# bluenote-1577/skani

Hardware: AMD Instinct MI355X
Metric: genome-pairs/sec (triangle, ~5 Mbp genomes) (higher is better)
Workload: dtype u64

## Files before the change

skani_amd/csrc/chain.hip:

```cpp
#include <algorithm>
#include <cmath>

#include "internal.h"

namespace skh {

#include "chain_types.h"
#include "chain_join.h"
#include "chain_chunk.h"
#include "chain_dp.h"
#include "chain_select.h"
#include "chain_stats.h"
#include "chain_estimate.h"

namespace {

static void genome_halves(const skh_sketch_set* S) {
    std::lock_guard<std::mutex> lk(S->cache_mu);
    if (S->halves.size() == S->n_genomes && S->n_genomes) return;
    S->halves.resize(S->n_genomes);
    for (uint32_t g = 0; g < S->n_genomes; g++) {
        skh_sketch_set::GenomeHalf& h = S->halves[g];
        h.n_pos = (uint32_t)(S->pos_off[g + 1] - S->pos_off[g]); h.pos0 = (uint32_t)S->pos_off[g];
        h.seed = S->p_seed.p + S->pos_off[g]; h.g = S->p_g.p + S->pos_off[g]; h.rep = S->p_rep.p; h.salt = S->salt[g];
// ... 230 lines not shown
            check_launch("join_fill");
        }
        std::vector<uint32_t> pa0(np + 1, 0), pc0(np + 1, 0), pi0(np + 1, 0), ps0(np + 1, 0);
        for (uint32_t i = 0; i < np; i++) {
            const uint32_t an = pair_anch[p0 + i];
            pa0[i + 1] = pa0[i] + an;
            pc0[i + 1] = pc0[i] + (an ? std::min(job.chunk_bound[p0 + i], an) : 0);
            const uint32_t icap = an / MIN_ANCHORS;
            pi0[i + 1] = pi0[i] + icap; ps0[i + 1] = ps0[i] + (icap >= big_min ? icap : 0);
            if (ps0[i + 1] < ps0[i]) throw Error("too many candidate intervals in one chain batch");
        }
        const uint32_t NC = pc0[np], NI = pi0[np], NS = ps0[np];
        std::vector<uint32_t> pfx(4 * ((size_t)np + 1));
        memcpy(pfx.data(), pa0.data(), ((size_t)np + 1) * 4); memcpy(pfx.data() + (np + 1), pc0.data(), ((size_t)np + 1) * 4);
        memcpy(pfx.data() + 2 * ((size_t)np + 1), pi0.data(), ((size_t)np + 1) * 4); memcpy(pfx.data() + 3 * ((size_t)np + 1), ps0.data(), ((size_t)np + 1) * 4);
        uint32_t* d_pa0 = upload(ctx, pfx); uint32_t* d_pc0 = d_pa0 + (np + 1); uint32_t* d_pi0 = d_pc0 + (np + 1); uint32_t* d_ps0 = d_pi0 + (np + 1);
        tr.mark("join_fill (+slots)");
        Co *anc_q, *anc_r;
        if constexpr (W::wide) {
            anc_q = ctx->arena.get<uint64_t>((size_t)NA + 16); anc_r = ctx->arena.get<uint64_t>((size_t)NA + 16);
            if (NA) {
                SKH_LAUNCH(widen_anchors_kernel, (NA + 255) / 256, 256, 0, ctx->stream, NA, np, (const uint32_t*)d_pa0, d_wide, (const uint32_t*)anc_q32, (const uint32_t*)anc_r32, anc_q, anc_r);
                check_launch("widen_anchors");
            }
        } else { anc_q = anc_q32; anc_r = anc_r32; }
        Chunk* chunks = ctx->arena.get<Chunk>(NC + 1); uint32_t* chunk_pair = ctx->arena.get<uint32_t>(NC + 1);
        uint32_t* n_chunks = ctx->arena.get<uint32_t>(np);
        SKH_LAUNCH(chunk_kernel<W>, (np + 3) / 4, 256, 0, ctx->stream, np, d_pairs, d_wide, (const uint32_t*)d_pa0, (const uint32_t*)(d_pair_anch + p0),
                   (const uint32_t*)d_pc0, (const Co*)anc_q, chunks, chunk_pair, n_chunks, d_err);
        check_launch("chunk");
        tr.mark("chunk");
        Interval* ivls = ctx->arena.get<Interval>(NI + 1); uint32_t* ivl_cnt = ctx->arena.get<uint32_t>(np);
        uint32_t* ivl_next = ctx->arena.get<uint32_t>(NI + 1); uint32_t* greedy_scratch = ctx->arena.get<uint32_t>((size_t)NS * GREEDY_BIG_WORDS + 1);
        uint32_t* chunk_head = ctx->arena.get<uint32_t>(NC + 1); uint32_t* n_acc = ctx->arena.get<uint32_t>(np);
        FillRegions stage_fills; stage_fills.add(ivl_cnt, np, 0u); stage_fills.add(chunk_head, (uint64_t)NC + 1, 0xFFFFFFFFu);
        bool stage_filled = false;
        const EmitCtxT<W> ec{anc_q, anc_r, d_pairs, d_wide, d_pc0, d_pi0, ivl_cnt, ivls, d_err};
        if (NC) {
            bool chained = false;
            if (band <= (W::wide ? 40u : 84u) && !(W::wide && ctx->tune.wide_sweep_dp)) {
                chained = true;
                constexpr int T = 64;
                const unsigned gt = (NC + T - 1) / T;
                const uint32_t ls = ctx->tune.chain_dp_lds_slots <= 1 ? 1u : 8u;
                const size_t n_spill = band + 1 > ls ? (size_t)(band + 1 - ls) * gt * T : 1;
                unsigned long long* spill_best = ctx->arena.get<unsigned long long>(n_spill); uint32_t* spill_rr = ctx->arena.get<uint32_t>(n_spill);
                uint4* emit_q = ctx->arena.get<uint4>((size_t)DP_EMIT_Q * gt * T);
                const unsigned ob = (NC + DP_ORDER_BLOCK - 1) / DP_ORDER_BLOCK;
                uint32_t* order = ctx->arena.get<uint32_t>(NC); uint32_t* ohist = ctx->arena.get<uint32_t>(2 * DP_ORDER_KEYS);
                stage_fills.add(ohist, 2 * DP_ORDER_KEYS, 0u); fill_regions(ctx, stage_fills); stage_filled = true;
                SKH_LAUNCH(dp_order_hist_kernel, ob, 256, 0, ctx->stream, NC, (const Chunk*)chunks, ohist);
                SKH_LAUNCH(dp_order_scatter_kernel, ob, 256, 0, ctx->stream, NC, (const Chunk*)chunks, (const uint32_t*)ohist, ohist + DP_ORDER_KEYS, order);
                check_launch("dp_order");
#define SKH_DPT2(NB, LS, EX) SKH_LAUNCH((chain_dp_thread_kernel<NB, T, LS, EX, W>), gt, T, 0, ctx->stream, NC, (const Chunk*)chunks, (const uint32_t*)chunk_pair, (const uint32_t*)order, band, ec, spill_best, spill_rr, emit_q, ls == 1 ? 1u : (uint32_t)DP_EMIT_Q)
#define SKH_DPT(NB, EX) do { if (ls == 1) SKH_DPT2(NB, 1, EX); else SKH_DPT2(NB, 8, EX); } while (0)
                if (band == 12) SKH_DPT(12, true); else if (band == 20) SKH_DPT(20, true); else if (band == 35) SKH_DPT(35, true);
                else if (band <= 12) SKH_DPT(12, false); else if (band <= 20) SKH_DPT(20, false); else if (band <= 28) SKH_DPT(28, false); else if (band <= 40) SKH_DPT(40, false);
                else if constexpr (!W::wide) { if (band == 83) SKH_DPT(83, true); else SKH_DPT(84, false); }
#undef SKH_DPT
#undef SKH_DPT2
                check_launch("chain_dp_thread");
            }
            if (!chained) {
                fill_regions(ctx, stage_fills); stage_filled = true;
                unsigned long long* best = ctx->arena.get<unsigned long long>((size_t)NA + 64);
                dzero(best, ((uint64_t)NA + 64) * 8, ctx->stream);
                const unsigned gb = (NC + 3) / 4;
                uint32_t* dp_state = band > 256 ? ctx->arena.get<uint32_t>(3 * (size_t)NA + 4) : nullptr;
#define SKH_DP(PB) SKH_LAUNCH((chain_dp_kernel<PB, W>), gb, 256, 0, ctx->stream, NC, (const Chunk*)chunks, band, (const Co*)anc_q, (const Co*)anc_r, best, dp_state)
                if (band <= 64) SKH_DP(1); else if (band <= 128) SKH_DP(2); else if (band <= 192) SKH_DP(3); else if (band <= 256) SKH_DP(4); else SKH_DP(0);
#undef SKH_DP
                check_launch("chain_dp");
                SKH_LAUNCH(interval_emit_kernel<W>, (NC + 3) / 4, 256, 0, ctx->stream, NC, (const Chunk*)chunks, (const unsigned long long*)best,
                           (const uint32_t*)chunk_pair, ec);
                check_launch("interval_emit");
            }
        }
        if (!stage_filled) fill_regions(ctx, stage_fills);
#define SKH_GREEDY(CAP) SKH_LAUNCH(greedy_fast_kernel<CAP>, np, 64, 0, ctx->stream, np, (const uint32_t*)g_order, (const uint32_t*)d_pi0, (const uint32_t*)d_pc0, \
                   (const uint32_t*)ivl_cnt, (const Interval*)ivls, ctx->tune.greedy_len_limit, big_min, ivl_next, chunk_head, n_acc); check_launch("greedy_fast")
        tr.mark("dp (+order sort)");
        uint32_t* g_keys = ctx->arena.get<uint32_t>(np); uint32_t* g_order = ctx->arena.get<uint32_t>(np);
        if (np <= GREEDY_ORDER_ONE_MAX) {
            SKH_LAUNCH(greedy_order_kernel, 1u, 1024, 0, ctx->stream, np, (const uint32_t*)ivl_cnt, g_order);
            check_launch("greedy_order");
        } else {
            SKH_LAUNCH(greedy_order_keys_kernel, (np + 255) / 256, 256, 0, ctx->stream, np, (const uint32_t*)ivl_cnt, g_keys, g_order);
            check_launch("greedy_order_keys");
            sort_pairs_u32_u32(ctx, g_keys, g_order, np, 16);
        }
        SKH_GREEDY(256); SKH_GREEDY(512); SKH_GREEDY(1024);
#undef SKH_GREEDY
        SKH_LAUNCH(greedy_kernel, (np + 3) / 4, 256, 0, ctx->stream, np, (const uint32_t*)d_pi0, (const uint32_t*)d_pc0,
                   (const uint32_t*)ivl_cnt, (const Interval*)ivls, big_min, ivl_next, chunk_head, n_acc);
        check_launch("greedy");
        if (NS) {
            SKH_LAUNCH(greedy_big_kernel, np, 1024, 0, ctx->stream, np, (const uint32_t*)d_pi0, (const uint32_t*)d_ps0, (const uint32_t*)d_pc0,
                       (const uint32_t*)ivl_cnt, (const Interval*)ivls, big_min, greedy_scratch, ivl_next, chunk_head, n_acc);
            check_launch("greedy_big");
        }
        tr.mark("greedy");
        double* chunk_est = ctx->arena.get<double>(NC + 1); uint32_t* chunk_w = ctx->arena.get<uint32_t>(NC + 1);
        uint4* chunk_sums = ctx->arena.get<uint4>(NC + 1);
        if (NC) {
            SKH_LAUNCH(chunk_stats_kernel<W>, (NC + 255) / 256, 256, 0, ctx->stream, NC, (const Chunk*)chunks, (const uint32_t*)chunk_pair, (const uint32_t*)chunk_head,
                       (const uint32_t*)ivl_next, (const Interval*)ivls, d_pairs, d_wide, (const unsigned long long*)imk, c, k, chunk_est, chunk_w, chunk_sums);
            check_launch("chunk_stats");
        }
        tr.mark("chunk_stats");
        FinalizeArgs fa{};
        fa.n_pairs = np; fa.c = c; fa.k = k; fa.min_af = mp.min_af; fa.both_min_af = mp.both_min_af; fa.robust = mp.robust; fa.median = mp.median;
// ... 165 lines not shown
```

skani_amd/csrc/chain_dp.h:

```cpp
#pragma once

template <class Co> struct Blk { Co q, r; uint32_t cr; int32_t score; uint32_t root, depth; };

template <int PB, class W>
__global__ __launch_bounds__(256) void chain_dp_kernel(uint32_t n_slots, const Chunk* chunks, uint32_t band, const typename W::Co* anc_q, const typename W::Co* anc_r, unsigned long long* best,
                                                       uint32_t* st ) {
    using Co = typename W::Co; using Blk = skh::Blk<Co>;
    const uint32_t slot = blockIdx.x * (blockDim.x >> 6) + (threadIdx.x >> 6);
    if (slot >= n_slots) return;
    const Chunk ck = chunks[slot];
    if (ck.a_end <= ck.a_begin) return;
    const int l = (int)lane_id();
    Blk prev[PB > 0 ? PB : 1];
#pragma unroll
    for (int b = 0; b < (PB > 0 ? PB : 1); b++) prev[b] = Blk{0, 0, 0, 0, 0, 0};
    for (uint32_t base = ck.a_begin; base < ck.a_end; base += 64) {
        const uint32_t t = base + (uint32_t)l;
        const bool valid = t < ck.a_end;
        Blk cur;
        Co av_q = 0, av_r = 0;
        if (valid) { av_q = anc_q[t]; av_r = anc_r[t]; }
        cur.q = av_q; cur.r = av_r >> 1; cur.cr = (uint32_t)(av_r & 1u);
        cur.score = 0; cur.root = t; cur.depth = 1;
        uint32_t ptr = t;
// ... 84 lines not shown
    iv.r0 = (uint32_t)((ra < rb ? ra : rb) - roff); iv.r1 = (uint32_t)((ra < rb ? rb : ra) - roff);
    iv.rctg = rctg; iv.qctg = ck.qctg; iv.chunk = slot - ec.pc0[p]; iv.rev = (uint32_t)(ar_r & 1u);
    ec.ivls[ec.pi0[p] + k] = iv;
}
template <class W>
__device__ __forceinline__ void dp_emit(const Chunk& ck, uint32_t slot, uint32_t p, uint32_t root, unsigned long long b, const EmitCtxT<W>& ec) {
    if (dp_keep(b)) dp_write(ck, slot, p, root, b, ec, atomicAdd(&ec.ivl_cnt[p], 1u));
}

constexpr uint32_t DP_ORDER_KEYS = 1024, DP_ORDER_BLOCK = 8192;
__device__ __forceinline__ uint32_t dp_order_key(const Chunk& c) { const uint32_t len = c.a_end - c.a_begin; return (DP_ORDER_KEYS - 1u) - (len >= DP_ORDER_KEYS - 1u ? DP_ORDER_KEYS - 1u : len); }
__global__ __launch_bounds__(256) void dp_order_hist_kernel(uint32_t n_slots, const Chunk* chunks, uint32_t* hist) {
    __shared__ uint32_t lh[DP_ORDER_KEYS];
    for (uint32_t x = threadIdx.x; x < DP_ORDER_KEYS; x += 256) lh[x] = 0;
    __syncthreads();
    const uint32_t e = (blockIdx.x + 1u) * DP_ORDER_BLOCK < n_slots ? (blockIdx.x + 1u) * DP_ORDER_BLOCK : n_slots;
    for (uint32_t i = blockIdx.x * DP_ORDER_BLOCK + threadIdx.x; i < e; i += 256) atomicAdd(&lh[dp_order_key(chunks[i])], 1u);
    __syncthreads();
    for (uint32_t x = threadIdx.x; x < DP_ORDER_KEYS; x += 256) if (lh[x]) atomicAdd(&hist[x], lh[x]);
}
__global__ __launch_bounds__(256) void dp_order_scatter_kernel(uint32_t n_slots, const Chunk* chunks, const uint32_t* hist, uint32_t* cursor, uint32_t* order) {
    __shared__ uint32_t base[DP_ORDER_KEYS], mine[DP_ORDER_KEYS]; __shared__ uint32_t wsum[4];
    const uint32_t t = threadIdx.x;
    uint32_t h[4], s = 0;
#pragma unroll
    for (int x = 0; x < 4; x++) { h[x] = hist[4 * t + x]; s += h[x]; mine[4 * t + x] = 0; }
    const uint32_t incl = wave_incl_scan(s);
    if ((t & 63u) == 63u) wsum[t >> 6] = incl;
    __syncthreads();
    uint32_t off = incl - s;
    for (uint32_t w = 0; w < (t >> 6); w++) off += wsum[w];
#pragma unroll
    for (int x = 0; x < 4; x++) { base[4 * t + x] = off; off += h[x]; }
    __syncthreads();
    constexpr int PER = DP_ORDER_BLOCK / 256;
    const uint32_t i0 = blockIdx.x * DP_ORDER_BLOCK + t;
    uint16_t k[PER], r[PER];
#pragma unroll
    for (int x = 0; x < PER; x++) { const uint32_t i = i0 + 256u * x; k[x] = 0xFFFF; if (i < n_slots) { k[x] = (uint16_t)dp_order_key(chunks[i]); r[x] = (uint16_t)atomicAdd(&mine[k[x]], 1u); } }
    __syncthreads();
#pragma unroll
    for (int x = 0; x < 4; x++) { const uint32_t c = 4 * t + x, n = mine[c]; if (n) base[c] += atomicAdd(&cursor[c], n); }
    __syncthreads();
#pragma unroll
    for (int x = 0; x < PER; x++) if (k[x] != 0xFFFF) order[base[k[x]] + r[x]] = i0 + 256u * x;
}

#ifndef DP_EMIT_Q
#define DP_EMIT_Q 6
#endif
#ifndef DP_LINE
#define DP_LINE 8
#endif
template <int NB, int T, uint32_t DP_LDS_SLOTS, bool EXACT, class W = Narrow>
__global__ __launch_bounds__(T) void chain_dp_thread_kernel(uint32_t n_slots, const Chunk* chunks, const uint32_t* chunk_pair, const uint32_t* order, uint32_t band,
                                                            EmitCtxT<W> ec, unsigned long long* spill_best, uint32_t* spill_rr, uint4* emit_q, uint32_t emit_cap) {
    using Co = typename W::Co;
    __shared__ unsigned long long lds_best[DP_LDS_SLOTS * T];
    __shared__ uint32_t lds_rr[DP_LDS_SLOTS * T];
    const uint32_t C = band + 1, tid = threadIdx.x;
    const uint32_t thr = blockIdx.x * T + tid;
    const uint32_t slot = thr < n_slots ? order[thr] : n_slots;
    const size_t n_thr = (size_t)gridDim.x * T;
    auto get_best = [&](uint32_t c) { return c < DP_LDS_SLOTS ? lds_best[c * T + tid] : spill_best[(size_t)(c - DP_LDS_SLOTS) * n_thr + thr]; };
    auto set_best = [&](uint32_t c, unsigned long long v) { if (c < DP_LDS_SLOTS) lds_best[c * T + tid] = v; else spill_best[(size_t)(c - DP_LDS_SLOTS) * n_thr + thr] = v; };
    auto get_rr = [&](uint32_t c) { return c < DP_LDS_SLOTS ? lds_rr[c * T + tid] : spill_rr[(size_t)(c - DP_LDS_SLOTS) * n_thr + thr]; };
    auto set_rr = [&](uint32_t c, uint32_t v) { if (c < DP_LDS_SLOTS) lds_rr[c * T + tid] = v; else spill_rr[(size_t)(c - DP_LDS_SLOTS) * n_thr + thr] = v; };
    Chunk ck{0, 0, 0, 0, 0, 0};
    if (slot < n_slots) ck = chunks[slot];
    const uint32_t n = ck.a_end - ck.a_begin;
    if (n >= MAX_CHUNK_ANCHORS) { atomicAdd(ec.err, 1u); return; }
    const uint32_t p = n ? chunk_pair[slot] : 0;
    uint32_t nq = 0;
    auto emit = [&](uint32_t root, unsigned long long b) {
        if (!dp_keep(b)) return;
        if (NB <= 40 && nq < emit_cap) { emit_q[(size_t)nq * n_thr + thr] = make_uint4(root, (uint32_t)b, (uint32_t)(b >> 32), 0u); nq++; }
        else dp_emit(ck, slot, p, root, b, ec);
    };
    unsigned long long free_mask = C >= 64 ? ~0ull : ((1ull << C) - 1ull);
    uint32_t rq[NB], rr[NB], rs[NB], rd[NB];
    uint32_t rh[W::wide ? NB : 1];
#pragma unroll
    for (int k = 0; k < NB; k++) { rq[k] = 0; rr[k] = 0; rs[k] = 0; rd[k] = 0; }
#pragma unroll
    for (int k = 0; k < (W::wide ? NB : 1); k++) rh[k] = 0;
    constexpr uint32_t LINE = DP_LINE;
    constexpr int APL = W::wide ? 2 : 4;
    constexpr int LQ = LINE / APL;
    __shared__ uint32_t lds_q[LINE * T], lds_r[LINE * T];
    __shared__ uint32_t lds_rh[W::wide ? LINE * T : 1];
    const uint32_t voff = ck.a_begin & (LINE - 1);
    const uint32_t vtot = n ? n + voff : 0;
    const Co* line_q = ec.anc_q + (ck.a_begin - voff); const Co* line_r = ec.anc_r + (ck.a_begin - voff);
    uint4 pq[LQ], pr[LQ];
#pragma unroll
    for (int j = 0; j < LQ; j++) { pq[j] = make_uint4(0, 0, 0, 0); pr[j] = make_uint4(0, 0, 0, 0); }
    if (vtot) {
#pragma unroll
        for (int j = 0; j < LQ; j++) { pq[j] = *(const uint4*)(line_q + APL * j); pr[j] = *(const uint4*)(line_r + APL * j); }
    }
    for (uint32_t v = 0;; v++) {
        const uint32_t kk = v & (LINE - 1);
        if (kk == 0) {
            if (__ballot(v < vtot) == 0) break;
#pragma unroll
            for (int j = 0; j < LQ; j++) {
                if constexpr (W::wide) {
                    lds_q[(2 * j + 0) * T + tid] = pq[j].x; lds_q[(2 * j + 1) * T + tid] = pq[j].z;
                    lds_r[(2 * j + 0) * T + tid] = pr[j].x; lds_r[(2 * j + 1) * T + tid] = pr[j].z;
                    lds_rh[(2 * j + 0) * T + tid] = pr[j].y; lds_rh[(2 * j + 1) * T + tid] = pr[j].w;
                } else {
                    lds_q[(4 * j + 0) * T + tid] = pq[j].x; lds_q[(4 * j + 1) * T + tid] = pq[j].y; lds_q[(4 * j + 2) * T + tid] = pq[j].z; lds_q[(4 * j + 3) * T + tid] = pq[j].w;
                    lds_r[(4 * j + 0) * T + tid] = pr[j].x; lds_r[(4 * j + 1) * T + tid] = pr[j].y; lds_r[(4 * j + 2) * T + tid] = pr[j].z; lds_r[(4 * j + 3) * T + tid] = pr[j].w;
                }
            }
            if (v + LINE < vtot) {
#pragma unroll
                for (int j = 0; j < LQ; j++) { pq[j] = *(const uint4*)(line_q + v + LINE + APL * j); pr[j] = *(const uint4*)(line_r + v + LINE + APL * j); }
            }
        }
        if (v < voff || v >= vtot) continue;
        const uint32_t i = v - voff;
        const uint2 a = make_uint2(lds_q[kk * T + tid], lds_r[kk * T + tid]);
        uint32_t q = a.x, r, sh = 0;
        if constexpr (W::wide) {
            const uint32_t ah = lds_rh[kk * T + tid];
            const uint64_t co = (((uint64_t)ah << 32) | a.y) >> 1, sv = (a.y & 1u) ? ~co : co;
            r = (uint32_t)sv; sh = (uint32_t)(sv >> 32);
        } else r = (a.y & 1u) ? ~(a.y >> 1) : (a.y >> 1);
        int32_t bscore = 0; uint32_t bdc = NONE;
        bool stop = false;
#pragma unroll
        for (int g = 0; g < NB; g += 4) {
            if (g > 0 && !stop) stop = __ballot((int32_t)(q - rq[g - 1]) < (int32_t)BP_CHAIN_BAND) == 0;
            if (!stop) {
#pragma unroll
                for (int k = g; k < g + 4 && k < NB; k++) {
                    if (EXACT || (uint32_t)k < band) {
                        const uint32_t dq1 = q - rq[k], dr1 = r - rr[k];
                        const uint32_t gap = abs_diff_u32(dr1, dq1);
                        const int32_t sc = (int32_t)(rs[k] - gap);
                        bool ok = (dq1 < BP_CHAIN_BAND) & (gap <= (uint32_t)MAX_GAP) & (sc > bscore);
                        if constexpr (W::wide) ok = ok & ((sh - rh[k]) == (r < rr[k] ? 1u : 0u));
                        bscore = ok ? sc : bscore; bdc = ok ? rd[k] : bdc;
                    }
                }
            }
        }
        uint32_t comp, depth;
        if (bdc != NONE) {
            comp = bdc & 0xFFu; depth = (bdc >> 8) + 1;
            set_rr(comp, get_rr(comp) + 1);
            const unsigned long long pay = best_payload((uint32_t)bscore, i, depth);
            if (pay > get_best(comp)) set_best(comp, pay);
        } else {
            comp = (uint32_t)__ffsll((long long)free_mask) - 1u; free_mask &= free_mask - 1ull; depth = 1;
            set_rr(comp, (i << 8) | 1u); set_best(comp, best_payload(0, i, 1));
        }
        uint32_t leaving = rd[NB - 1];
        if (!EXACT) {
#pragma unroll
            for (int k = 0; k < NB; k++) leaving = ((uint32_t)k == band - 1) ? rd[k] : leaving;
        }
        if (i >= band) {
            const uint32_t c_old = leaving & 0xFFu;
            const uint32_t v = get_rr(c_old) - 1u;
            set_rr(c_old, v);
            if ((v & 0xFFu) == 0) { emit(v >> 8, get_best(c_old)); free_mask |= 1ull << c_old; }
        }
#pragma unroll
        for (int k = NB - 1; k > 0; k--) { rq[k] = rq[k - 1]; rr[k] = rr[k - 1]; rs[k] = rs[k - 1]; rd[k] = rd[k - 1]; }
        if constexpr (W::wide) {
#pragma unroll
            for (int k = NB - 1; k > 0; k--) rh[k] = rh[k - 1];
            rh[0] = sh + (r == 0xFFFFFFFFu ? 1u : 0u);
        }
        rq[0] = q + 1u; rr[0] = r + 1u; rs[0] = (uint32_t)(bscore + ANCHOR_SCORE); rd[0] = (depth << 8) | comp;
    }
    const uint32_t live = n < band ? n : band;
#pragma unroll
    for (int k = 0; k < NB; k++) {
        if ((uint32_t)k < live) {
            const uint32_t c_old = rd[k] & 0xFFu;
            const uint32_t v = get_rr(c_old) - 1u;
            set_rr(c_old, v);
            if ((v & 0xFFu) == 0) emit(v >> 8, get_best(c_old));
        }
    }
    if (NB <= 40 && nq) {
        const uint32_t k0 = atomicAdd(&ec.ivl_cnt[p], nq);
        for (uint32_t e = 0; e < nq; e++) {
            const uint4 r = emit_q[(size_t)e * n_thr + thr];
            dp_write(ck, slot, p, r.x, ((unsigned long long)r.z << 32) | r.y, ec, k0 + e);
        }
    }
}

template <class W>
__global__ __launch_bounds__(256) void interval_emit_kernel(uint32_t n_slots, const Chunk* chunks, const unsigned long long* best, const uint32_t* chunk_pair, EmitCtxT<W> ec) {
    const uint32_t slot = blockIdx.x * (blockDim.x >> 6) + (threadIdx.x >> 6);
    if (slot >= n_slots) return;
    const Chunk ck = chunks[slot];
    if (ck.a_end <= ck.a_begin) return;
    const uint32_t p = chunk_pair[slot];
    if (ck.a_end - ck.a_begin >= MAX_CHUNK_ANCHORS) { if (lane_id() == 0) atomicAdd(ec.err, 1u); return; }
    for (uint32_t i = ck.a_begin + lane_id(); i < ck.a_end; i += 64) {
        const unsigned long long b = best[i];
        if (b != 0) dp_emit(ck, slot, p, i - ck.a_begin, b, ec);
    }
}
```

skani_amd/csrc/dev.h:

```cpp
#pragma once
#include <cstddef>
#include <cstdint>
#include <cstdio>
#include <cstring>
#include <stdexcept>
#include <string>

namespace skh {
struct Error : std::runtime_error { using std::runtime_error::runtime_error; };
struct PeerError : Error { using Error::Error; };
}

#ifdef SKANI_EMU
#include "emu_dev.h"
#else
#include <hip/hip_runtime.h>
typedef hipStream_t devStream_t;
#define SKH_LAUNCH(kernel, grid, block, smem, stream, ...) \
    hipLaunchKernelGGL(kernel, dim3(grid), dim3(block), (smem), (stream), __VA_ARGS__)
#define SKH_DYN_SMEM(name) extern __shared__ __attribute__((aligned(16))) char name[]

namespace skh {

inline void hip_check(hipError_t e, const char* what) {
    if (e != hipSuccess) throw Error(std::string(what) + ": " + hipGetErrorString(e));
}
void* dmalloc(size_t n);
void dfree(void* p);
void dcache_trim();
void dcache_stats(size_t* live_bytes, size_t* idle_bytes);
size_t device_memory_free();
struct PinRing {
    char* p = nullptr; size_t cap = 0, off = 0; bool tried = false;
    hipStream_t s0 = nullptr, s1 = nullptr;
    bool used0 = false, used1 = false;
    ~PinRing() { if (p) (void)hipHostFree(p); }
};
inline PinRing*& pin_ring_of_thread() { static thread_local PinRing* r = nullptr; return r; }
struct PinScope {
    PinRing* prev; int prev_dev = -1;
    PinScope(int device, PinRing* ring) : prev(pin_ring_of_thread()) {
        int cur = -1;
        if (hipGetDevice(&cur) != hipSuccess) { (void)hipGetLastError(); cur = -1; }
        if (cur != device) { (void)hipSetDevice(device); prev_dev = cur; }
        pin_ring_of_thread() = ring;
    }
    ~PinScope() { pin_ring_of_thread() = prev; if (prev_dev >= 0) (void)hipSetDevice(prev_dev); }
};
inline bool pageable_direct() { static const bool on = [] { const char* v = getenv("SKH_TUNE_PAGEABLE_DIRECT"); return v && *v && *v != '0'; }(); return on; }
inline bool pin_ring_ready(PinRing* r, devStream_t s) {
    constexpr size_t PIN_RING = (size_t)8 << 20;
    if (!r || !(s == r->s0 || s == r->s1)) return false;
    if (!r->tried) { r->tried = true; void* q = nullptr; if (hipHostMalloc(&q, PIN_RING, hipHostMallocPortable) == hipSuccess) { r->p = (char*)q; r->cap = PIN_RING; } else (void)hipGetLastError(); }
    return r->p != nullptr;
}
inline char* pin_ring_take(PinRing* r, size_t n, hipStream_t s) {
    const size_t need = (n + 255) & ~(size_t)255;
    if (r->off + need > r->cap) {
        if (r->used0) hip_check(hipStreamSynchronize(r->s0), "pinned ring wrap");
        if (r->used1) hip_check(hipStreamSynchronize(r->s1), "pinned ring wrap");
        r->used0 = r->used1 = false; r->off = 0;
    }
    if (s == r->s0) r->used0 = true; else r->used1 = true;
    char* p = r->p + r->off; r->off += need; return p;
}
constexpr size_t PIN_CHUNK = (size_t)4 << 20;
inline void h2d(void* d, const void* h, size_t n, devStream_t s) {
    if (!n) return;
    constexpr size_t PIN_MAX = (size_t)1 << 20;
    PinRing* r = pin_ring_of_thread();
    if ((n <= PIN_MAX || !pageable_direct()) && pin_ring_ready(r, s)) {
        for (size_t at = 0; at < n; at += PIN_CHUNK) {
            const size_t m = n - at < PIN_CHUNK ? n - at : PIN_CHUNK;
// ... 33 lines not shown
inline void check_launch(const char* what) { hip_check(hipGetLastError(), what); }
inline void device_sync_all() noexcept { (void)hipDeviceSynchronize(); }

inline void dev_open(int device, devStream_t* s0, devStream_t* s1) {
    int n = 0;
    hip_check(hipGetDeviceCount(&n), "hipGetDeviceCount");
    if (device < 0 || device >= n) throw Error("no such HIP device (this library has no CPU path)");
    hip_check(hipSetDevice(device), "hipSetDevice");
    hip_check(hipStreamCreateWithFlags(s0, hipStreamNonBlocking), "hipStreamCreate");
    hip_check(hipStreamCreateWithFlags(s1, hipStreamNonBlocking), "hipStreamCreate");
}
inline void dev_drain(int device, devStream_t s0, devStream_t s1) noexcept { (void)hipSetDevice(device); (void)hipStreamSynchronize(s0); (void)hipStreamSynchronize(s1); }
inline void dev_close(devStream_t s0, devStream_t s1) noexcept { (void)hipStreamDestroy(s0); (void)hipStreamDestroy(s1); }

struct DevEvent {
    hipEvent_t e = nullptr;
    DevEvent() { hip_check(hipEventCreate(&e), "hipEventCreate"); }
    ~DevEvent() { if (e) (void)hipEventDestroy(e); }
    DevEvent(const DevEvent&) = delete; DevEvent& operator=(const DevEvent&) = delete;
    DevEvent(DevEvent&& o) noexcept : e(o.e) { o.e = nullptr; }
    void record(devStream_t s) { hip_check(hipEventRecord(e, s), "hipEventRecord"); }
    void wait() { hip_check(hipEventSynchronize(e), "hipEventSynchronize"); }
    bool done() { const hipError_t r = hipEventQuery(e); if (r == hipSuccess) return true; (void)hipGetLastError(); return false; }
    void make_wait(devStream_t s) { hip_check(hipStreamWaitEvent(s, e, 0), "hipStreamWaitEvent"); }
    static float ms(const DevEvent& a, const DevEvent& b) { float t = 0; hip_check(hipEventElapsedTime(&t, a.e, b.e), "hipEventElapsedTime"); return t; }
};

template <class K> inline void kernel_allow_lds(K kernel, size_t bytes) {
    hip_check(hipFuncSetAttribute((const void*)kernel, hipFuncAttributeMaxDynamicSharedMemorySize, (int)bytes), "LDS size attribute");
}

#if defined(__HIP_DEVICE_COMPILE__)
template <class T> using GlobalPtr = const T __attribute__((address_space(1)))*;
#else
template <class T> using GlobalPtr = const T*;
#endif
template <class T> __device__ __forceinline__ GlobalPtr<T> global_of(const T* p) { return (GlobalPtr<T>)p; }

__device__ __forceinline__ int wave_readlane(int v, int uniform_lane) { return __builtin_amdgcn_readlane(v, __builtin_amdgcn_readfirstlane(uniform_lane)); }
__device__ __forceinline__ void wave_sync_mem() { __builtin_amdgcn_fence(__ATOMIC_SEQ_CST, "workgroup"); __builtin_amdgcn_wave_barrier(); }
__device__ __forceinline__ void block_fence() { __builtin_amdgcn_fence(__ATOMIC_SEQ_CST, "workgroup"); }
__device__ __forceinline__ uint32_t abs_diff_u32(uint32_t a, uint32_t b) { uint32_t d; asm("v_sad_u32 %0, %1, %2, 0" : "=v"(d) : "v"(a), "v"(b)); return d; }
__device__ __forceinline__ uint32_t lane_next(uint32_t v) { return (uint32_t)__builtin_amdgcn_update_dpp((int)v, (int)v, 0x130, 0xF, 0xF, false); }
__device__ __forceinline__ uint32_t lane_prev(uint32_t v) { return (uint32_t)__builtin_amdgcn_update_dpp((int)v, (int)v, 0x138, 0xF, 0xF, false); }
__device__ __forceinline__ unsigned wave_incl_scan(unsigned v) {
    asm volatile("s_nop 1\n\tv_add_u32_dpp %0, %0, %0 row_shr:1 row_mask:0xf bank_mask:0xf\n\t"
                 "s_nop 1\n\tv_add_u32_dpp %0, %0, %0 row_shr:2 row_mask:0xf bank_mask:0xf\n\t"
                 "s_nop 1\n\tv_add_u32_dpp %0, %0, %0 row_shr:4 row_mask:0xf bank_mask:0xf\n\t"
                 "s_nop 1\n\tv_add_u32_dpp %0, %0, %0 row_shr:8 row_mask:0xf bank_mask:0xf\n\t"
                 "s_nop 1\n\tv_add_u32_dpp %0, %0, %0 row_bcast:15 row_mask:0xa bank_mask:0xf\n\t"
                 "s_nop 1\n\tv_add_u32_dpp %0, %0, %0 row_bcast:31 row_mask:0xc bank_mask:0xf" : "+v"(v));
    return v;
}
__device__ __forceinline__ unsigned long long wave_clock() { return __builtin_readcyclecounter(); }
__device__ __forceinline__ void wait_for_value(uint32_t v) { asm volatile("" ::"v"(v)); }
__device__ __forceinline__ uint32_t xcc_id() { uint32_t x; asm volatile("s_getreg_b32 %0, hwreg(HW_REG_XCC_ID)" : "=s"(x)); return x & 0xFu; }
__device__ __forceinline__ uint32_t load_past_l1(const uint32_t* p) { return __hip_atomic_load(p, __ATOMIC_RELAXED, __HIP_MEMORY_SCOPE_AGENT); }
__device__ __forceinline__ void atomic_inc_xcd_local(uint32_t* p) { __hip_atomic_fetch_add(p, 1u, __ATOMIC_RELAXED, __HIP_MEMORY_SCOPE_WORKGROUP); }

#define SKH_SEED_DROP_NOTE() ((void)0)
__device__ __forceinline__ unsigned long long wave_mask_ge(uint32_t a, uint32_t b) { return __builtin_amdgcn_uicmp(a, b, 35 ); }
__device__ __forceinline__ void or_in_lanes(uint32_t& v, unsigned long long lanes, uint32_t bits) {
    unsigned long long save;
    asm volatile("s_mov_b64 %1, exec\n\ts_mov_b64 exec, %2\n\tv_or_b32 %0, %3, %0\n\ts_mov_b64 exec, %1" : "+v"(v), "=&s"(save) : "s"(lanes), "s"(bits));
}
__device__ __forceinline__ uint32_t funnel_shr(uint32_t hi, uint32_t lo, uint32_t sh) { return __builtin_amdgcn_alignbit(hi, lo, sh); }
template <int SH> __device__ __forceinline__ uint64_t shl_add_u64(uint64_t a, uint64_t b) {
    uint64_t d; asm("v_lshl_add_u64 %0, %1, %3, %2" : "=v"(d) : "v"(a), "v"(b), "n"(SH)); return d;
}
__device__ __forceinline__ uint64_t seed_hash(uint32_t seed) {
    const uint64_t p = (uint64_t)seed * 0x200001ull;
    const uint32_t plo = (uint32_t)p, phi = (uint32_t)(p >> 32);
    const uint32_t lo2 = plo ^ __builtin_amdgcn_alignbit(phi, plo, 24);
    const uint32_t hi2 = phi ^ 0xFFFFFF00u;
    const uint64_t q = (uint64_t)lo2 * 265u;
    uint32_t hi3; asm("v_mad_i32_i24 %0, %1, %2, %3" : "=v"(hi3) : "v"(hi2), "s"(265u), "v"((uint32_t)(q >> 32)));
    uint64_t key = ((uint64_t)hi3 << 32) | (uint32_t)q;
    key ^= key >> 14;
    key = shl_add_u64<4>(key, shl_add_u64<2>(key, key));
    key ^= key >> 28;
    return shl_add_u64<0>(key << 31, key);
}
__device__ __forceinline__ uint32_t seed_probe(uint32_t seed) {
    const uint64_t p = (uint64_t)seed * 0x200001ull;
    const uint32_t plo = (uint32_t)p, phi = (uint32_t)(p >> 32);
    const uint32_t lo2 = plo ^ __builtin_amdgcn_alignbit(phi, plo, 24);
    const uint32_t hi2 = phi ^ 0xFFFFFF00u;
    const uint64_t q = (uint64_t)lo2 * 265u;
    uint32_t hi3; asm("v_mad_i32_i24 %0, %1, %2, %3" : "=v"(hi3) : "v"(hi2), "s"(265u), "v"((uint32_t)(q >> 32)));
    uint64_t key = ((uint64_t)hi3 << 32) | (uint32_t)q;
    key ^= key >> 14;
    key = shl_add_u64<4>(key, shl_add_u64<2>(key, key));
    uint64_t sh; asm("v_lshrrev_b64 %0, 28, %1" : "=v"(sh) : "v"(key));
    uint32_t nlo, nhi;
    asm("v_xnor_b32 %0, %1, %2" : "=v"(nlo) : "v"((uint32_t)key), "v"((uint32_t)sh));
    asm("v_xnor_b32 %0, %1, %2" : "=v"(nhi) : "v"((uint32_t)(key >> 32)), "v"((uint32_t)(sh >> 32)));
    return nhi + __builtin_amdgcn_alignbit(nhi, nlo, 1);
}

}
#endif

namespace skh {

struct PinBuf {
    void* p = nullptr; size_t cap = 0;
// ... 32 lines not shown
```

Before: 41.49 million.

## Process anchors in groups of four with direct uint4 loads in chain DP

For narrow coordinates with bands up to 40, the per-thread chain DP now reads four anchors per 16-byte global load, double-buffered in registers, instead of staging lines through LDS. The register window is widened by three so the shifts happen once per group of four anchors. The live components at the end are flushed by walking the free mask rather than the band window. It also forces a minimum waves-per-EU occupancy hint for small exact bands and keeps the slot lookup out of registers by recomputing indices. The risks are higher register pressure and unaligned group handling at chunk boundaries.

Result: slower. 40.85 million (-1.6%).

```diff
diff --git a/skani_amd/csrc/chain.hip b/skani_amd/csrc/chain.hip
--- a/skani_amd/csrc/chain.hip
+++ b/skani_amd/csrc/chain.hip
@@ -306,11 +306,11 @@
                 SKH_LAUNCH(dp_order_hist_kernel, ob, 256, 0, ctx->stream, NC, (const Chunk*)chunks, ohist);
                 SKH_LAUNCH(dp_order_scatter_kernel, ob, 256, 0, ctx->stream, NC, (const Chunk*)chunks, (const uint32_t*)ohist, ohist + DP_ORDER_KEYS, order);
                 check_launch("dp_order");
-#define SKH_DPT2(NB, LS, EX) SKH_LAUNCH((chain_dp_thread_kernel<NB, T, LS, EX, W>), gt, T, 0, ctx->stream, NC, (const Chunk*)chunks, (const uint32_t*)chunk_pair, (const uint32_t*)order, band, ec, spill_best, spill_rr, emit_q, ls == 1 ? 1u : (uint32_t)DP_EMIT_Q)
-#define SKH_DPT(NB, EX) do { if (ls == 1) SKH_DPT2(NB, 1, EX); else SKH_DPT2(NB, 8, EX); } while (0)
-                if (band == 12) SKH_DPT(12, true); else if (band == 20) SKH_DPT(20, true); else if (band == 35) SKH_DPT(35, true);
-                else if (band <= 12) SKH_DPT(12, false); else if (band <= 20) SKH_DPT(20, false); else if (band <= 28) SKH_DPT(28, false); else if (band <= 40) SKH_DPT(40, false);
-                else if constexpr (!W::wide) { if (band == 83) SKH_DPT(83, true); else SKH_DPT(84, false); }
+#define SKH_DPT2(NB, LS, EX, GS) SKH_LAUNCH((chain_dp_thread_kernel<NB, T, LS, EX, W, (W::wide ? 1 : GS)>), gt, T, 0, ctx->stream, NC, (const Chunk*)chunks, (const uint32_t*)chunk_pair, (const uint32_t*)order, band, ec, spill_best, spill_rr, emit_q, ls == 1 ? 1u : (uint32_t)DP_EMIT_Q)
+#define SKH_DPT(NB, EX, GS) do { if (ls == 1) SKH_DPT2(NB, 1, EX, GS); else SKH_DPT2(NB, 8, EX, GS); } while (0)
+                if (band == 12) SKH_DPT(12, true, 4); else if (band == 20) SKH_DPT(20, true, 4); else if (band == 35) SKH_DPT(35, true, 4);
+                else if (band <= 12) SKH_DPT(12, false, 4); else if (band <= 20) SKH_DPT(20, false, 4); else if (band <= 28) SKH_DPT(28, false, 4); else if (band <= 40) SKH_DPT(40, false, 4);
+                else if constexpr (!W::wide) { if (band == 83) SKH_DPT(83, true, 1); else SKH_DPT(84, false, 1); }
 #undef SKH_DPT
 #undef SKH_DPT2
                 check_launch("chain_dp_thread");
diff --git a/skani_amd/csrc/chain_dp.h b/skani_amd/csrc/chain_dp.h
--- a/skani_amd/csrc/chain_dp.h
+++ b/skani_amd/csrc/chain_dp.h
@@ -160,8 +160,9 @@
 #ifndef DP_LINE
 #define DP_LINE 8
 #endif
-template <int NB, int T, uint32_t DP_LDS_SLOTS, bool EXACT, class W = Narrow>
-__global__ __launch_bounds__(T) void chain_dp_thread_kernel(uint32_t n_slots, const Chunk* chunks, const uint32_t* chunk_pair, const uint32_t* order, uint32_t band,
+template <int V> struct DpIdx { static constexpr int value = V; };
+template <int NB, int T, uint32_t DP_LDS_SLOTS, bool EXACT, class W = Narrow, int GS = 1>
+__global__ __launch_bounds__(T) SKH_MIN_WAVES_PER_SIMD((GS == 4 && NB <= 20 && EXACT) ? 4 : 1) void chain_dp_thread_kernel(uint32_t n_slots, const Chunk* chunks, const uint32_t* chunk_pair, const uint32_t* order, uint32_t band,
                                                             EmitCtxT<W> ec, unsigned long long* spill_best, uint32_t* spill_rr, uint4* emit_q, uint32_t emit_cap) {
     using Co = typename W::Co;
     __shared__ unsigned long long lds_best[DP_LDS_SLOTS * T];
@@ -170,10 +171,11 @@
     const uint32_t thr = blockIdx.x * T + tid;
     const uint32_t slot = thr < n_slots ? order[thr] : n_slots;
     const size_t n_thr = (size_t)gridDim.x * T;
-    auto get_best = [&](uint32_t c) { return c < DP_LDS_SLOTS ? lds_best[c * T + tid] : spill_best[(size_t)(c - DP_LDS_SLOTS) * n_thr + thr]; };
-    auto set_best = [&](uint32_t c, unsigned long long v) { if (c < DP_LDS_SLOTS) lds_best[c * T + tid] = v; else spill_best[(size_t)(c - DP_LDS_SLOTS) * n_thr + thr] = v; };
-    auto get_rr = [&](uint32_t c) { return c < DP_LDS_SLOTS ? lds_rr[c * T + tid] : spill_rr[(size_t)(c - DP_LDS_SLOTS) * n_thr + thr]; };
-    auto set_rr = [&](uint32_t c, uint32_t v) { if (c < DP_LDS_SLOTS) lds_rr[c * T + tid] = v; else spill_rr[(size_t)(c - DP_LDS_SLOTS) * n_thr + thr] = v; };
+    auto col = [&]() { if constexpr (GS == 4) return blockIdx.x * T + reg_local(tid); else return thr; };
+    auto get_best = [&](uint32_t c) { return c < DP_LDS_SLOTS ? lds_best[c * T + tid] : spill_best[(size_t)(c - DP_LDS_SLOTS) * n_thr + col()]; };
+    auto set_best = [&](uint32_t c, unsigned long long v) { if (c < DP_LDS_SLOTS) lds_best[c * T + tid] = v; else spill_best[(size_t)(c - DP_LDS_SLOTS) * n_thr + col()] = v; };
+    auto get_rr = [&](uint32_t c) { return c < DP_LDS_SLOTS ? lds_rr[c * T + tid] : spill_rr[(size_t)(c - DP_LDS_SLOTS) * n_thr + col()]; };
+    auto set_rr = [&](uint32_t c, uint32_t v) { if (c < DP_LDS_SLOTS) lds_rr[c * T + tid] = v; else spill_rr[(size_t)(c - DP_LDS_SLOTS) * n_thr + col()] = v; };
     Chunk ck{0, 0, 0, 0, 0, 0};
     if (slot < n_slots) ck = chunks[slot];
     const uint32_t n = ck.a_end - ck.a_begin;
@@ -182,124 +184,207 @@
     uint32_t nq = 0;
     auto emit = [&](uint32_t root, unsigned long long b) {
         if (!dp_keep(b)) return;
-        if (NB <= 40 && nq < emit_cap) { emit_q[(size_t)nq * n_thr + thr] = make_uint4(root, (uint32_t)b, (uint32_t)(b >> 32), 0u); nq++; }
-        else dp_emit(ck, slot, p, root, b, ec);
+        if (NB <= 40 && nq < emit_cap) { emit_q[(size_t)nq * n_thr + col()] = make_uint4(root, (uint32_t)b, (uint32_t)(b >> 32), 0u); nq++; }
+        else if constexpr (GS == 1) dp_emit(ck, slot, p, root, b, ec);
+        else { const uint32_t s = order[col()]; dp_emit(chunks[s], s, chunk_pair[s], root, b, ec); }
     };
     unsigned long long free_mask = C >= 64 ? ~0ull : ((1ull << C) - 1ull);
-    uint32_t rq[NB], rr[NB], rs[NB], rd[NB];
-    uint32_t rh[W::wide ? NB : 1];
-#pragma unroll
-    for (int k = 0; k < NB; k++) { rq[k] = 0; rr[k] = 0; rs[k] = 0; rd[k] = 0; }
-#pragma unroll
-    for (int k = 0; k < (W::wide ? NB : 1); k++) rh[k] = 0;
-    constexpr uint32_t LINE = DP_LINE;
-    constexpr int APL = W::wide ? 2 : 4;
-    constexpr int LQ = LINE / APL;
-    __shared__ uint32_t lds_q[LINE * T], lds_r[LINE * T];
-    __shared__ uint32_t lds_rh[W::wide ? LINE * T : 1];
-    const uint32_t voff = ck.a_begin & (LINE - 1);
-    const uint32_t vtot = n ? n + voff : 0;
-    const Co* line_q = ec.anc_q + (ck.a_begin - voff); const Co* line_r = ec.anc_r + (ck.a_begin - voff);
-    uint4 pq[LQ], pr[LQ];
-#pragma unroll
-    for (int j = 0; j < LQ; j++) { pq[j] = make_uint4(0, 0, 0, 0); pr[j] = make_uint4(0, 0, 0, 0); }
-    if (vtot) {
-#pragma unroll
-        for (int j = 0; j < LQ; j++) { pq[j] = *(const uint4*)(line_q + APL * j); pr[j] = *(const uint4*)(line_r + APL * j); }
-    }
-    for (uint32_t v = 0;; v++) {
-        const uint32_t kk = v & (LINE - 1);
-        if (kk == 0) {
-            if (__ballot(v < vtot) == 0) break;
-#pragma unroll
-            for (int j = 0; j < LQ; j++) {
-                if constexpr (W::wide) {
-                    lds_q[(2 * j + 0) * T + tid] = pq[j].x; lds_q[(2 * j + 1) * T + tid] = pq[j].z;
-                    lds_r[(2 * j + 0) * T + tid] = pr[j].x; lds_r[(2 * j + 1) * T + tid] = pr[j].z;
-                    lds_rh[(2 * j + 0) * T + tid] = pr[j].y; lds_rh[(2 * j + 1) * T + tid] = pr[j].w;
-                } else {
-                    lds_q[(4 * j + 0) * T + tid] = pq[j].x; lds_q[(4 * j + 1) * T + tid] = pq[j].y; lds_q[(4 * j + 2) * T + tid] = pq[j].z; lds_q[(4 * j + 3) * T + tid] = pq[j].w;
-                    lds_r[(4 * j + 0) * T + tid] = pr[j].x; lds_r[(4 * j + 1) * T + tid] = pr[j].y; lds_r[(4 * j + 2) * T + tid] = pr[j].z; lds_r[(4 * j + 3) * T + tid] = pr[j].w;
-                }
-            }
-            if (v + LINE < vtot) {
-#pragma unroll
-                for (int j = 0; j < LQ; j++) { pq[j] = *(const uint4*)(line_q + v + LINE + APL * j); pr[j] = *(const uint4*)(line_r + v + LINE + APL * j); }
-            }
-        }
-        if (v < voff || v >= vtot) continue;
-        const uint32_t i = v - voff;
-        const uint2 a = make_uint2(lds_q[kk * T + tid], lds_r[kk * T + tid]);
-        uint32_t q = a.x, r, sh = 0;
-        if constexpr (W::wide) {
-            const uint32_t ah = lds_rh[kk * T + tid];
-            const uint64_t co = (((uint64_t)ah << 32) | a.y) >> 1, sv = (a.y & 1u) ? ~co : co;
-            r = (uint32_t)sv; sh = (uint32_t)(sv >> 32);
-        } else r = (a.y & 1u) ? ~(a.y >> 1) : (a.y >> 1);
-        int32_t bscore = 0; uint32_t bdc = NONE;
-        bool stop = false;
-#pragma unroll
-        for (int g = 0; g < NB; g += 4) {
-            if (g > 0 && !stop) stop = __ballot((int32_t)(q - rq[g - 1]) < (int32_t)BP_CHAIN_BAND) == 0;
-            if (!stop) {
-#pragma unroll
-                for (int k = g; k < g + 4 && k < NB; k++) {
-                    if (EXACT || (uint32_t)k < band) {
-                        const uint32_t dq1 = q - rq[k], dr1 = r - rr[k];
-                        const uint32_t gap = abs_diff_u32(dr1, dq1);
-                        const int32_t sc = (int32_t)(rs[k] - gap);
-                        bool ok = (dq1 < BP_CHAIN_BAND) & (gap <= (uint32_t)MAX_GAP) & (sc > bscore);
-                        if constexpr (W::wide) ok = ok & ((sh - rh[k]) == (r < rr[k] ? 1u : 0u));
-                        bscore = ok ? sc : bscore; bdc = ok ? rd[k] : bdc;
+    if constexpr (GS == 4) {
+        static_assert(!W::wide, "groups of four anchors: 32-bit coordinates only (a 16-byte load holds two 64-bit anchors)");
+        using Mask = std::conditional_t<(NB < 32), uint32_t, unsigned long long>;
+        Mask fm = (Mask)free_mask;
+        uint32_t rq[NB + 3], rr[NB + 3], rs[NB + 3], rd[NB + 3];
+#pragma unroll
+        for (int k = 0; k < NB + 3; k++) { rq[k] = 0; rr[k] = 0; rs[k] = 0; rd[k] = 0; }
+        const uint32_t a_begin = ck.a_begin, a_end = ck.a_end;
+        const uint32_t g0 = a_begin >> 2;
+        const uint4* const grp_q = (const uint4*)ec.anc_q; const uint4* const grp_r = (const uint4*)ec.anc_r;
+        uint4 nxt_q = make_uint4(0, 0, 0, 0), nxt_r = make_uint4(0, 0, 0, 0);
+        if (n) { nxt_q = grp_q[g0]; nxt_r = grp_r[g0]; }
+        uint32_t tq = 0, tr = 0, ts = 0, td = 0;
+        auto sub = [&](auto sidx, uint32_t at, uint32_t aq, uint32_t ar) {
+            constexpr int S = decltype(sidx)::value, B = 3 - S;
+            if (at + (uint32_t)S < a_begin || at + (uint32_t)S >= a_end) return;
+            const uint32_t i = at + (uint32_t)S - a_begin;
+            const uint32_t q = aq, r = (ar & 1u) ? ~(ar >> 1) : (ar >> 1);
+            int32_t bscore = 0; uint32_t bdc = NONE;
+            bool stop = false;
+#pragma unroll
+            for (int g = 0; g < NB; g += 4) {
+                if (g > 0 && !stop) stop = __ballot((int32_t)(q - rq[B + g - 1]) < (int32_t)BP_CHAIN_BAND) == 0;
+                if (!stop) {
+#pragma unroll
+                    for (int k = g; k < g + 4 && k < NB; k++) {
+                        if (EXACT || (uint32_t)k < band) {
+                            const uint32_t dq1 = q - rq[B + k], dr1 = r - rr[B + k];
+                            const uint32_t gap = abs_diff_u32(dr1, dq1);
+                            const int32_t sc = (int32_t)(rs[B + k] - gap);
+                            const bool ok = (dq1 < BP_CHAIN_BAND) & (gap <= (uint32_t)MAX_GAP) & (sc > bscore);
+                            bscore = ok ? sc : bscore; bdc = ok ? rd[B + k] : bdc;
+                        }
                     }
                 }
             }
-        }
-        uint32_t comp, depth;
-        if (bdc != NONE) {
-            comp = bdc & 0xFFu; depth = (bdc >> 8) + 1;
-            set_rr(comp, get_rr(comp) + 1);
-            const unsigned long long pay = best_payload((uint32_t)bscore, i, depth);
-            if (pay > get_best(comp)) set_best(comp, pay);
-        } else {
-            comp = (uint32_t)__ffsll((long long)free_mask) - 1u; free_mask &= free_mask - 1ull; depth = 1;
-            set_rr(comp, (i << 8) | 1u); set_best(comp, best_payload(0, i, 1));
-        }
-        uint32_t leaving = rd[NB - 1];
-        if (!EXACT) {
-#pragma unroll
-            for (int k = 0; k < NB; k++) leaving = ((uint32_t)k == band - 1) ? rd[k] : leaving;
-        }
-        if (i >= band) {
-            const uint32_t c_old = leaving & 0xFFu;
-            const uint32_t v = get_rr(c_old) - 1u;
-            set_rr(c_old, v);
-            if ((v & 0xFFu) == 0) { emit(v >> 8, get_best(c_old)); free_mask |= 1ull << c_old; }
-        }
-#pragma unroll
-        for (int k = NB - 1; k > 0; k--) { rq[k] = rq[k - 1]; rr[k] = rr[k - 1]; rs[k] = rs[k - 1]; rd[k] = rd[k - 1]; }
-        if constexpr (W::wide) {
-#pragma unroll
-            for (int k = NB - 1; k > 0; k--) rh[k] = rh[k - 1];
-            rh[0] = sh + (r == 0xFFFFFFFFu ? 1u : 0u);
-        }
-        rq[0] = q + 1u; rr[0] = r + 1u; rs[0] = (uint32_t)(bscore + ANCHOR_SCORE); rd[0] = (depth << 8) | comp;
-    }
-    const uint32_t live = n < band ? n : band;
-#pragma unroll
-    for (int k = 0; k < NB; k++) {
-        if ((uint32_t)k < live) {
-            const uint32_t c_old = rd[k] & 0xFFu;
-            const uint32_t v = get_rr(c_old) - 1u;
-            set_rr(c_old, v);
-            if ((v & 0xFFu) == 0) emit(v >> 8, get_best(c_old));
+            uint32_t comp, depth;
+            if (bdc != NONE) {
+                comp = bdc & 0xFFu; depth = (bdc >> 8) + 1;
+                set_rr(comp, get_rr(comp) + 1);
+                const unsigned long long pay = best_payload((uint32_t)bscore, i, depth);
+                if (pay > get_best(comp)) set_best(comp, pay);
+            } else {
+                comp = (uint32_t)__ffsll((long long)(unsigned long long)fm) - 1u; fm &= fm - (Mask)1; depth = 1;
+                set_rr(comp, (i << 8) | 1u); set_best(comp, best_payload(0, i, 1));
+            }
+            uint32_t leaving = rd[B + NB - 1];
+            if (!EXACT) {
+#pragma unroll
+                for (int k = 0; k < NB; k++) leaving = ((uint32_t)k == band - 1) ? rd[B + k] : leaving;
+            }
+            if (i >= band) {
+                const uint32_t c_old = leaving & 0xFFu;
+                const uint32_t x = get_rr(c_old) - 1u;
+                set_rr(c_old, x);
+                if ((x & 0xFFu) == 0) { emit(x >> 8, get_best(c_old)); fm |= (Mask)1 << c_old; }
+            }
+            const uint32_t eq = q + 1u, er = r + 1u, es = (uint32_t)(bscore + ANCHOR_SCORE), ed = (depth << 8) | comp;
+            if constexpr (S < 3) { rq[2 - S] = eq; rr[2 - S] = er; rs[2 - S] = es; rd[2 - S] = ed; }
+            else { tq = eq; tr = er; ts = es; td = ed; }
+        };
+        for (uint32_t v = 0;; v += 4) {
+            const uint32_t at = (a_begin & ~3u) + v;
+            if (__ballot(at < a_end) == 0) break;
+            const uint4 cq = nxt_q, cr = nxt_r;
+            sub(DpIdx<0>{}, at, cq.x, cr.x);
+            sub(DpIdx<1>{}, at, cq.y, cr.y);
+            if (at + 4 < a_end) { nxt_q = grp_q[(at >> 2) + 1]; nxt_r = grp_r[(at >> 2) + 1]; }
+            sub(DpIdx<2>{}, at, cq.z, cr.z);
+            sub(DpIdx<3>{}, at, cq.w, cr.w);
+#pragma unroll
+            for (int k = NB + 2; k > 3; k--) { rq[k] = rq[k - 4]; rr[k] = rr[k - 4]; rs[k] = rs[k - 4]; rd[k] = rd[k - 4]; }
+            rq[3] = tq; rr[3] = tr; rs[3] = ts; rd[3] = td;
+        }
+        for (unsigned long long m = ~(unsigned long long)fm & free_mask; m; m &= m - 1ull) {
+            const uint32_t c = (uint32_t)__ffsll((long long)m) - 1u;
+            emit(get_rr(c) >> 8, get_best(c));
+        }
+    } else {
+        uint32_t rq[NB], rr[NB], rs[NB], rd[NB];
+        uint32_t rh[W::wide ? NB : 1];
+    #pragma unroll
+        for (int k = 0; k < NB; k++) { rq[k] = 0; rr[k] = 0; rs[k] = 0; rd[k] = 0; }
+    #pragma unroll
+        for (int k = 0; k < (W::wide ? NB : 1); k++) rh[k] = 0;
+        constexpr uint32_t LINE = DP_LINE;
+        constexpr int APL = W::wide ? 2 : 4;
+        constexpr int LQ = LINE / APL;
+        __shared__ uint32_t lds_q[LINE * T], lds_r[LINE * T];
+        __shared__ uint32_t lds_rh[W::wide ? LINE * T : 1];
+        const uint32_t voff = ck.a_begin & (LINE - 1);
+        const uint32_t vtot = n ? n + voff : 0;
+        const Co* line_q = ec.anc_q + (ck.a_begin - voff); const Co* line_r = ec.anc_r + (ck.a_begin - voff);
+        uint4 pq[LQ], pr[LQ];
+    #pragma unroll
+        for (int j = 0; j < LQ; j++) { pq[j] = make_uint4(0, 0, 0, 0); pr[j] = make_uint4(0, 0, 0, 0); }
+        if (vtot) {
+    #pragma unroll
+            for (int j = 0; j < LQ; j++) { pq[j] = *(const uint4*)(line_q + APL * j); pr[j] = *(const uint4*)(line_r + APL * j); }
+        }
+        for (uint32_t v = 0;; v++) {
+            const uint32_t kk = v & (LINE - 1);
+            if (kk == 0) {
+                if (__ballot(v < vtot) == 0) break;
+    #pragma unroll
+                for (int j = 0; j < LQ; j++) {
+                    if constexpr (W::wide) {
+                        lds_q[(2 * j + 0) * T + tid] = pq[j].x; lds_q[(2 * j + 1) * T + tid] = pq[j].z;
+                        lds_r[(2 * j + 0) * T + tid] = pr[j].x; lds_r[(2 * j + 1) * T + tid] = pr[j].z;
+                        lds_rh[(2 * j + 0) * T + tid] = pr[j].y; lds_rh[(2 * j + 1) * T + tid] = pr[j].w;
+                    } else {
+                        lds_q[(4 * j + 0) * T + tid] = pq[j].x; lds_q[(4 * j + 1) * T + tid] = pq[j].y; lds_q[(4 * j + 2) * T + tid] = pq[j].z; lds_q[(4 * j + 3) * T + tid] = pq[j].w;
+                        lds_r[(4 * j + 0) * T + tid] = pr[j].x; lds_r[(4 * j + 1) * T + tid] = pr[j].y; lds_r[(4 * j + 2) * T + tid] = pr[j].z; lds_r[(4 * j + 3) * T + tid] = pr[j].w;
+                    }
+                }
+                if (v + LINE < vtot) {
+    #pragma unroll
+                    for (int j = 0; j < LQ; j++) { pq[j] = *(const uint4*)(line_q + v + LINE + APL * j); pr[j] = *(const uint4*)(line_r + v + LINE + APL * j); }
+                }
+            }
+            if (v < voff || v >= vtot) continue;
+            const uint32_t i = v - voff;
+            const uint2 a = make_uint2(lds_q[kk * T + tid], lds_r[kk * T + tid]);
+            uint32_t q = a.x, r, sh = 0;
+            if constexpr (W::wide) {
+                const uint32_t ah = lds_rh[kk * T + tid];
+                const uint64_t co = (((uint64_t)ah << 32) | a.y) >> 1, sv = (a.y & 1u) ? ~co : co;
+                r = (uint32_t)sv; sh = (uint32_t)(sv >> 32);
+            } else r = (a.y & 1u) ? ~(a.y >> 1) : (a.y >> 1);
+            int32_t bscore = 0; uint32_t bdc = NONE;
+            bool stop = false;
+    #pragma unroll
+            for (int g = 0; g < NB; g += 4) {
+                if (g > 0 && !stop) stop = __ballot((int32_t)(q - rq[g - 1]) < (int32_t)BP_CHAIN_BAND) == 0;
+                if (!stop) {
+    #pragma unroll
+                    for (int k = g; k < g + 4 && k < NB; k++) {
+                        if (EXACT || (uint32_t)k < band) {
+                            const uint32_t dq1 = q - rq[k], dr1 = r - rr[k];
+                            const uint32_t gap = abs_diff_u32(dr1, dq1);
+                            const int32_t sc = (int32_t)(rs[k] - gap);
+                            bool ok = (dq1 < BP_CHAIN_BAND) & (gap <= (uint32_t)MAX_GAP) & (sc > bscore);
+                            if constexpr (W::wide) ok = ok & ((sh - rh[k]) == (r < rr[k] ? 1u : 0u));
+                            bscore = ok ? sc : bscore; bdc = ok ? rd[k] : bdc;
+                        }
+                    }
+                }
+            }
+            uint32_t comp, depth;
+            if (bdc != NONE) {
+                comp = bdc & 0xFFu; depth = (bdc >> 8) + 1;
+                set_rr(comp, get_rr(comp) + 1);
+                const unsigned long long pay = best_payload((uint32_t)bscore, i, depth);
+                if (pay > get_best(comp)) set_best(comp, pay);
+            } else {
+                comp = (uint32_t)__ffsll((long long)free_mask) - 1u; free_mask &= free_mask - 1ull; depth = 1;
+                set_rr(comp, (i << 8) | 1u); set_best(comp, best_payload(0, i, 1));
+            }
+            uint32_t leaving = rd[NB - 1];
+            if (!EXACT) {
+    #pragma unroll
+                for (int k = 0; k < NB; k++) leaving = ((uint32_t)k == band - 1) ? rd[k] : leaving;
+            }
+            if (i >= band) {
+                const uint32_t c_old = leaving & 0xFFu;
+                const uint32_t v = get_rr(c_old) - 1u;
+                set_rr(c_old, v);
+                if ((v & 0xFFu) == 0) { emit(v >> 8, get_best(c_old)); free_mask |= 1ull << c_old; }
+            }
+    #pragma unroll
+            for (int k = NB - 1; k > 0; k--) { rq[k] = rq[k - 1]; rr[k] = rr[k - 1]; rs[k] = rs[k - 1]; rd[k] = rd[k - 1]; }
+            if constexpr (W::wide) {
+    #pragma unroll
+                for (int k = NB - 1; k > 0; k--) rh[k] = rh[k - 1];
+                rh[0] = sh + (r == 0xFFFFFFFFu ? 1u : 0u);
+            }
+            rq[0] = q + 1u; rr[0] = r + 1u; rs[0] = (uint32_t)(bscore + ANCHOR_SCORE); rd[0] = (depth << 8) | comp;
+        }
+        const uint32_t live = n < band ? n : band;
+    #pragma unroll
+        for (int k = 0; k < NB; k++) {
+            if ((uint32_t)k < live) {
+                const uint32_t c_old = rd[k] & 0xFFu;
+                const uint32_t v = get_rr(c_old) - 1u;
+                set_rr(c_old, v);
+                if ((v & 0xFFu) == 0) emit(v >> 8, get_best(c_old));
+            }
         }
     }
     if (NB <= 40 && nq) {
-        const uint32_t k0 = atomicAdd(&ec.ivl_cnt[p], nq);
+        uint32_t ws = slot, wp = p; Chunk wck = ck;
+        if constexpr (GS == 4) { ws = order[thr]; wp = chunk_pair[ws]; wck = chunks[ws]; }
+        const uint32_t k0 = atomicAdd(&ec.ivl_cnt[wp], nq);
         for (uint32_t e = 0; e < nq; e++) {
             const uint4 r = emit_q[(size_t)e * n_thr + thr];
-            dp_write(ck, slot, p, r.x, ((unsigned long long)r.z << 32) | r.y, ec, k0 + e);
+            dp_write(wck, ws, wp, r.x, ((unsigned long long)r.z << 32) | r.y, ec, k0 + e);
         }
     }
 }
diff --git a/skani_amd/csrc/dev.h b/skani_amd/csrc/dev.h
--- a/skani_amd/csrc/dev.h
+++ b/skani_amd/csrc/dev.h
@@ -13,12 +13,15 @@
 
 #ifdef SKANI_EMU
 #include "emu_dev.h"
+#define SKH_MIN_WAVES_PER_SIMD(n)
+namespace skh { inline uint32_t reg_local(uint32_t v) { return v; } }
 #else
 #include <hip/hip_runtime.h>
 typedef hipStream_t devStream_t;
 #define SKH_LAUNCH(kernel, grid, block, smem, stream, ...) \
     hipLaunchKernelGGL(kernel, dim3(grid), dim3(block), (smem), (stream), __VA_ARGS__)
 #define SKH_DYN_SMEM(name) extern __shared__ __attribute__((aligned(16))) char name[]
+#define SKH_MIN_WAVES_PER_SIMD(n) __attribute__((amdgpu_waves_per_eu(n)))
 
 namespace skh {
 
@@ -158,6 +161,7 @@
                  "s_nop 1\n\tv_add_u32_dpp %0, %0, %0 row_bcast:31 row_mask:0xc bank_mask:0xf" : "+v"(v));
     return v;
 }
+__device__ __forceinline__ uint32_t reg_local(uint32_t v) { asm volatile("" : "+v"(v)); return v; }
 __device__ __forceinline__ unsigned long long wave_clock() { return __builtin_readcyclecounter(); }
 __device__ __forceinline__ void wait_for_value(uint32_t v) { asm volatile("" ::"v"(v)); }
 __device__ __forceinline__ uint32_t xcc_id() { uint32_t x; asm volatile("s_getreg_b32 %0, hwreg(HW_REG_XCC_ID)" : "=s"(x)); return x & 0xFu; }
```
